# sefffal/Octofitter.jl

Hardware: AMD Instinct MI355X
Metric: epoch-likelihood evals/sec (fwd+grad), 1e4 epochs x 1e4 walkers (higher is better)
Workload: dtype f64; 1 GPU; config3: 1 planet, 10000 RA/Dec epochs x 10000 walkers in total (10000 walkers split over 1 GPUs: 10000 walkers/GPU), fwd+reverse-grad, inputs and outputs resident in HBM (PCIe-inclusive rate: value_pcie_inclusive); walkers_per_gpu=10000, walkers_total=10000, rows=10000, parallelism=walkers sharded x1, dataset replicated, no data-path collective

## Files before the change

### __graft_entry__.py

```python
from __future__ import annotations

import functools
import importlib.util
import os
import shutil
import subprocess
import sys
from pathlib import Path

ROOT = Path(__file__).resolve().parent
PKG_DIR = ROOT / "octofitter.jl_amd"
PKG_NAME = "octofitter_jl_amd"
CSRC = PKG_DIR / "csrc"
LIB = PKG_DIR / "lib" / "liboctofitter_hip.so"

HIPCC_FLAGS = [
    "--offload-arch=gfx950", "-O3", "-std=c++17", "-fPIC",
    "-ffp-contract=on",
    "-fno-gpu-rdc",
    "-mllvm", "-structurizecfg-skip-uniform-regions",
    "-Wall", "-Wno-unused-function",
]


# ... 25 lines not shown
    return all(Path(s).stat().st_mtime <= t for s in sources)


def build_hip(force=False):
    from concurrent.futures import ThreadPoolExecutor
    hipcc = shutil.which("hipcc") or "/opt/rocm/bin/hipcc"
    sources = sorted(CSRC.glob("*.hip"))
    headers = sorted(CSRC.glob("*.h")) + [ROOT / "include" / "octofitter_hip.h"]
    LIB.parent.mkdir(parents=True, exist_ok=True)
    objdir = CSRC / "build"
    objdir.mkdir(exist_ok=True)
    cflags = [f for f in HIPCC_FLAGS if f != "-shared"]

    def compile_one(src):
        obj = objdir / (src.stem + ".o")
        if not force and _newer(obj, [src] + headers):
            return obj
        subprocess.run([hipcc, *cflags, f"-I{ROOT / 'include'}", f"-I{CSRC}", "-c", "-o", str(obj), str(src)], check=True)
        return obj

    with ThreadPoolExecutor(max_workers=min(len(sources), os.cpu_count() or 1)) as ex:
        objs = list(ex.map(compile_one, sources))
    if force or not _newer(LIB, objs):
        subprocess.run([hipcc, "--offload-arch=gfx950", "-shared", "-fPIC", "-fno-gpu-rdc", "-o", str(LIB), *map(str, objs)], check=True)
    return LIB


COMPANIONS = {
    "draws": dict(header="octofitter_hip_draws.h", links_main=True, main_headers=True),
    "predict": dict(header="octofitter_hip_predict.h", links_main=True, main_headers=True),
    "pointwise": dict(header="octofitter_hip_pointwise.h", links_main=True, main_headers=True),
    "psis": dict(header="octofitter_hip_psis.h", links_main=False, main_headers=False),
}


def companion_lib(name) -> Path:
    return PKG_DIR / "lib" / f"liboctofitter_hip_{name}.so"


def build_companion(name, force=False):
    row = COMPANIONS[name]
    hipcc = shutil.which("hipcc") or "/opt/rocm/bin/hipcc"
    src_dir, shared, out = CSRC / name, CSRC / "companion", companion_lib(name)
    sources = sorted(src_dir.glob("*.hip"))
    headers = sorted(src_dir.glob("*.h")) + sorted(shared.glob("*.h")) + (sorted(CSRC.glob("*.h")) if row["main_headers"] else []) + \
        [ROOT / "include" / "octofitter_hip.h", ROOT / "include" / row["header"]]
    if row["links_main"] and not LIB.exists():
# ... 78 lines not shown
```

### octofitter.jl_amd/csrc/octo_api.hip

```cpp
#define OCTO_API_TU 1
#include "octo_host.h"
#include "octo_tile.h"

using namespace octo;

namespace octo {

std::atomic<uint64_t> g_dataset_serial{1};

int fail(octo_ctx* ctx, int code, const std::string& msg) {
    if (ctx) ctx->err = msg;
    return code;
}

int busy(octo_ctx* ctx, const char* what) {
    if (ctx->pending.active) return fail(ctx, OCTO_EINVAL, std::string(what) + ": an octo_eval_begin of this context has not been ended");
    return OCTO_OK;
}


DevConsts dev_consts(const octo_consts& c) {
    DevConsts d;
    d.k_yr = c.kepler_year_to_julian_day; d.yd = c.year2day_julian; d.au2m = c.au2m; d.sec2yr = c.sec2year_julian;
    d.mas_per_au_per_plx = c.rad2as / c.pc2au;
// ... 152 lines not shown
            t_o = std::min<int64_t>(std::max<int64_t>(t_o, 1), std::max<int64_t>(1, n / (rows_min * wpb)));
            const int64_t rows_per_task = (n + t_o - 1) / t_o;
            chunk = (rows_per_task + wpb - 1) / wpb;
        }
        const int64_t span = chunk * wpb;
        bool even = n > 1;
        {
            double smin = INFINITY, smax = 0.0;
            for (int64_t r = 1; r < n; ++r) { smin = std::min(smin, (double)ds->h_step[o][r]); smax = std::max(smax, (double)ds->h_step[o][r]); }
            even = even && std::isfinite(smax) && smin > 0.0 && smax - smin <= 1.0e-7 * smax;
        }
        for (int64_t r0 = 0; r0 < n; r0 += span) {
            Task t;
            std::memset(&t, 0, sizeof(t));
            t.obs = o; t.row0 = (int32_t)r0; t.nrows = (int32_t)std::min<int64_t>(span, n - r0); t.chunk = (int32_t)chunk;
            {
                double km = 0.0;
                for (int64_t r = r0; r < r0 + t.nrows; ++r)
                    if ((r - r0) % chunk != 0) km = std::max(km, (double)ds->h_step[o][r]);
                float f = (float)km;
                if ((double)f < km) f = std::nextafterf(f, INFINITY);
                t.key_max = std::isfinite(km) ? f : INFINITY;
                t.dm_uniform = (even && std::isfinite(km) && km > 0.0) ? f : 0.0f;
            }
            tt.h_tasks.push_back(t);
            double a = 0.0, b = 0.0;
            for (int64_t r = r0; r < r0 + t.nrows; ++r) { a += ds->h_rowconst_pre[o][r]; b += ds->h_rowconst_raw[o][r]; }
            cpre.push_back(a); craw.push_back(b);
        }
    }
    tt.n_tasks = (int)tt.h_tasks.size();
    {
        std::vector<int32_t> range(2 * std::max(ds->n_obs, 1), 0);
        std::vector<double> opre(std::max(ds->n_obs, 1), 0.0), oraw(std::max(ds->n_obs, 1), 0.0);
        int t = 0;
        for (int o = 0; o < ds->n_obs; ++o) {
            range[2 * o] = t;
            while (t < tt.n_tasks && tt.h_tasks[t].obs == o) { opre[o] += cpre[t]; oraw[o] += craw[t]; ++t; }
            range[2 * o + 1] = t;
        }
        HIPCHK(ctx, hipMalloc((void**)&tt.d_obs_range, sizeof(int32_t) * range.size()));
        HIPCHK(ctx, hipMalloc((void**)&tt.d_obs_const_pre, sizeof(double) * opre.size()));
        HIPCHK(ctx, hipMalloc((void**)&tt.d_obs_const_raw, sizeof(double) * oraw.size()));
        HIPCHK(ctx, hipMemcpy(tt.d_obs_range, range.data(), sizeof(int32_t) * range.size(), hipMemcpyHostToDevice));
        HIPCHK(ctx, hipMemcpy(tt.d_obs_const_pre, opre.data(), sizeof(double) * opre.size(), hipMemcpyHostToDevice));
        HIPCHK(ctx, hipMemcpy(tt.d_obs_const_raw, oraw.data(), sizeof(double) * oraw.size(), hipMemcpyHostToDevice));
// ... 192 lines not shown
        }
    }
    if (hipMalloc((void**)&ctx->d_counters, sizeof(int32_t) * SMALL_W) != hipSuccess ||
        hipMemset(ctx->d_counters, 0, sizeof(int32_t) * SMALL_W) != hipSuccess) {
        (void)hipFree(ctx->d_sctab); (void)hipStreamDestroy(ctx->stream); (void)hipEventDestroy(ctx->ev_order);
        delete ctx;
        return OCTO_ENOMEM;
    }
    if (hipHostMalloc((void**)&ctx->h_flags, sizeof(uint64_t) * (SMALL_W + 32), hipHostMallocMapped | hipHostMallocPortable | hipHostMallocCoherent) != hipSuccess) {
        (void)hipFree(ctx->d_counters); (void)hipFree(ctx->d_sctab); (void)hipStreamDestroy(ctx->stream); (void)hipEventDestroy(ctx->ev_order);
        delete ctx;
        return OCTO_ENOMEM;
    }
    std::memset(ctx->h_flags, 0, sizeof(uint64_t) * (SMALL_W + 32));
    if (const char* ev = std::getenv("OCTO_SMALL_W")) { ctx->small_w = std::min(std::max(std::atoi(ev), 0), SMALL_W); ctx->small_w_model = 0; }
    if (const char* ev = std::getenv("OCTO_MAPPED_W")) ctx->mapped_w = std::min(std::max(std::atoi(ev), 0), SMALL_W);
    if (const char* ev = std::getenv("OCTO_FLAG_W")) ctx->flag_w = std::min(std::max(std::atoi(ev), 0), SMALL_W);
    ctx->env_small_blocks = env_int("OCTO_SMALL_BLOCKS"); ctx->env_small_min_span = env_int("OCTO_SMALL_MIN_SPAN");
    ctx->env_stage_bytes = env_int("OCTO_STAGE_BYTES"); ctx->env_chunk = env_int("OCTO_CHUNK"); ctx->env_rounds = env_int("OCTO_ROUNDS"); ctx->env_rv_cost = env_int("OCTO_RV_COST"); ctx->env_kind_all = env_int("OCTO_KIND_ALL"); ctx->env_mainp_tpb = env_int("OCTO_MAINP_TPB");
    if (const char* ev = std::getenv("OCTO_WIDE")) ctx->env_wide = std::atoi(ev);
    if (const char* ev = std::getenv("OCTO_FIN_FUSED")) ctx->env_no_fin_fused = std::atoi(ev) ? 0 : 1;
    if (const char* ev = std::getenv("OCTO_WARM")) { ctx->env_warm = std::atoi(ev); ctx->opt_warm = ctx->env_warm ? 1 : 0; }
    if (const char* ev = std::getenv("OCTO_WARM_NEWTON")) ctx->env_warm_newton = std::atoi(ev) ? 1 : 0;
    if (const char* ev = std::getenv("OCTO_WARM_NEWTON_MID")) ctx->env_warm_newton_mid = std::atoi(ev) ? 1 : 0;
    if (const char* ev = std::getenv("OCTO_TILE_SORT")) ctx->tile_mode = std::min(std::max(std::atoi(ev), 0), 2);
    if (const char* ev = std::getenv("OCTO_TILE_MIN_W")) ctx->tile_min_w = std::max<int64_t>(std::atoll(ev), 64);
    *out = ctx;
    return OCTO_OK;
}

int32_t octo_ctx_destroy(octo_ctx* ctx) {
    if (!ctx) return OCTO_OK;
    (void)hipSetDevice(ctx->device);
    if (ctx->comm) (void)octo_comm_destroy(ctx);
    (void)hipDeviceSynchronize();
    if (ctx->stream) (void)hipStreamDestroy(ctx->stream);
    if (ctx->ev_order) (void)hipEventDestroy(ctx->ev_order);
    free_retired(ctx);
    for (auto& t : ctx->tables) free_table(t);
    for (auto& e : ctx->ev_pool) { (void)hipEventDestroy(e.first); (void)hipEventDestroy(e.second); }
    (void)hipFree(ctx->d_wc); (void)hipFree(ctx->d_valid); (void)hipFree(ctx->d_partials); (void)hipFree(ctx->d_marg); (void)hipFree(ctx->d_sctab); (void)hipFree(ctx->d_extra); (void)hipFree(ctx->d_counters);
    (void)hipHostFree(ctx->h_in); (void)hipHostFree(ctx->h_out); (void)hipHostFree(ctx->h_flags);
    (void)hipFree(ctx->d_in); (void)hipFree(ctx->d_out);
    (void)hipFree(ctx->d_perm); (void)hipHostFree(ctx->h_tile_stats);
    for (void* q : ctx->retired_host) (void)hipHostFree(q);
    if (ctx->ev_tile) (void)hipEventDestroy(ctx->ev_tile);
// ... 61 lines not shown
        case OCTO_OPT_TILE_SORT: *value_out = ctx->tile_mode; return OCTO_OK;
        case OCTO_OPT_TILE_MIN_WALKERS: *value_out = ctx->tile_min_w; return OCTO_OK;
        default: return OCTO_EINVAL;
    }
}

int32_t octo_dataset_create(octo_ctx* ctx, const octo_obs_desc* obs, int32_t n_obs,
                            const octo_planet_desc* planets, int32_t n_planets, octo_dataset** out) {
    if (!ctx || !out || n_obs < 0 || (n_obs > 0 && !obs) || !planets) return fail(ctx, OCTO_EINVAL, "octo_dataset_create: null argument");
    *out = nullptr;
    if (n_planets < 1) return fail(ctx, OCTO_EINVAL, "octo_dataset_create: a dataset needs at least one planet");
    if (n_planets > MAXP) return fail(ctx, OCTO_ENOTSUP, "octo_dataset_create: 1.." + std::to_string(MAXP) + " planets supported");
    for (int p = 0; p < n_planets; ++p)
        if (planets[p].orbit_kind != OCTO_ORBIT_VISUAL_KEP && planets[p].orbit_kind != OCTO_ORBIT_RADVEL &&
            planets[p].orbit_kind != OCTO_ORBIT_THIELE_INNES && planets[p].orbit_kind != OCTO_ORBIT_KEP)
            return fail(ctx, OCTO_EINVAL, "octo_dataset_create: unknown orbit kind");
    HIPCHK(ctx, hipSetDevice(ctx->device));
    octo_dataset* ds = new (std::nothrow) octo_dataset();
    if (!ds) return fail(ctx, OCTO_ENOMEM, "octo_dataset_create: host allocation failed");
    ds->device = ctx->device; ds->n_obs = n_obs; ds->n_planets = n_planets;
    ds->serial = g_dataset_serial.fetch_add(1);
    for (int p = 0; p < n_planets; ++p) ds->planets[p] = planets[p];
    auto bail = [&](int code, const std::string& msg) { octo_dataset_destroy(ds); return fail(ctx, code, msg); };
    ds->h_obs.resize(n_obs); ds->h_rowconst_pre.resize(n_obs); ds->h_rowconst_raw.resize(n_obs); ds->h_step.resize(n_obs);
    for (int o = 0; o < n_obs; ++o) {
        const octo_obs_desc& d = obs[o];
        if (d.kind < 0 || d.kind >= OCTO_N_KINDS) return bail(OCTO_EINVAL, "octo_dataset_create: unknown observation kind");
        if (d.n_epochs < 0 || d.n_epochs > 0x7fffffff) return bail(OCTO_EINVAL, "octo_dataset_create: bad n_epochs");
        if (d.kind == OCTO_HGCA) {
            if (d.n_epochs > 0 && (!d.epoch || !d.y1 || !d.y2)) return bail(OCTO_EINVAL, "octo_dataset_create: missing column");
            if (!d.extra || d.n_extra != OCTO_HGCA_N_EXTRA) return bail(OCTO_EINVAL, "octo_dataset_create: OCTO_HGCA needs extra[15]");
            for (int p = 0; p < n_planets; ++p)
                if (planets[p].orbit_kind != OCTO_ORBIT_RADVEL && planets[p].orbit_kind != OCTO_ORBIT_KEP && !planets[p].has_mass)
                    return bail(OCTO_EINVAL, "octo_dataset_create: OCTO_HGCA needs a mass on every Visual{KepOrbit} / ThieleInnesOrbit planet");
            for (int k = 0; k < 3; ++k)
                if (!(d.extra[5 * k + 2] > 0.0) || !(d.extra[5 * k + 3] > 0.0) || !(std::fabs(d.extra[5 * k + 4]) < 1.0))
                    return bail(OCTO_EINVAL, "octo_dataset_create: OCTO_HGCA covariance is not positive definite");
            const int64_t n = d.n_epochs;
            std::vector<double> raw((size_t)std::max<int64_t>(n, 1) * ROW_STRIDE, 0.0);
            for (int64_t r = 0; r < n; ++r) {
                const int ax = (int)d.y1[r], ms = (int)d.y2[r];
                if ((ax != OCTO_HGCA_RA && ax != OCTO_HGCA_DEC) || (ms != OCTO_HGCA_HIP && ms != OCTO_HGCA_GAIA))
                    return bail(OCTO_EINVAL, "octo_dataset_create: OCTO_HGCA rows need y1 in {RA, DEC}, y2 in {HIP, GAIA}");
                if (!std::isfinite(d.epoch[r])) return bail(OCTO_EINVAL, "octo_dataset_create: OCTO_HGCA epochs must be finite");
                raw[(size_t)r * ROW_STRIDE] = d.epoch[r]; raw[(size_t)r * ROW_STRIDE + 1] = ax; raw[(size_t)r * ROW_STRIDE + 2] = ms;
            }
            DevObs& h = ds->h_obs[o];
// ... 55 lines not shown
                if (d.cor && !(std::fabs(c) <= 1.0 - 1e-5))
                    return bail(OCTO_EINVAL, "octo_dataset_create: correlation values may not be well-specified");
                a[2] = b[2] = d.y2[r]; a[3] = s1; a[4] = s2; a[5] = c;
                const double omc = 1.0 - c * c;
                b[3] = 1.0 / (s1 * s1 * omc); b[4] = 1.0 / (s2 * s2 * omc); b[5] = -c / (s1 * s2 * omc);
                ds->h_rowconst_pre[o][r] = -LOG2PI - 0.5 * std::log(s1 * s1 * s2 * s2 * omc);
                ds->h_rowconst_raw[o][r] = -LOG2PI;
            } else {
                const double s = d.s1[r];
                a[2] = s; b[2] = 1.0 / (s * s);
                if (has_basis) {
                    if (!std::isfinite(d.extra[r])) return bail(OCTO_EINVAL, "octo_dataset_create: table " + std::to_string(o) + " row " + std::to_string(r) + ": trend basis must be finite");
                    a[3] = d.extra[r];
                }
                if (d.kind == OCTO_RV_ABS_MARG) {
                    ds->h_rowconst_pre[o][r] = -std::log(TWO_PI * s * s);
                    ds->h_rowconst_raw[o][r] = 0.0;
                } else {
                    ds->h_rowconst_pre[o][r] = -0.5 * (LOG2PI + std::log(s * s));
                    ds->h_rowconst_raw[o][r] = -0.5 * LOG2PI;
                }
            }
        }
        double dm_max = 0.0;
        std::vector<double> steps;
        steps.reserve((size_t)std::max<int64_t>(n, 1));
        for (int64_t r = 0; r < n; ++r) {
            const double dm = r > 0 ? TWO_PI * (d.epoch[r] - d.epoch[r - 1]) : 0.0;
            double key = std::fabs(dm);
            if (r > 0) { dm_max = std::max(dm_max, key); steps.push_back(key); }
            ds->h_step[o][r] = std::isfinite(key) ? key : INFINITY;
            if (r == 0 || (r % WARM_RESTART) == 0 || !std::isfinite(key)) key = INFINITY;
            raw[(size_t)r * ROW_STRIDE + 6] = pre[(size_t)r * ROW_STRIDE + 6] = dm;
            raw[(size_t)r * ROW_STRIDE + 7] = pre[(size_t)r * ROW_STRIDE + 7] = key;
        }
        DevObs& h = ds->h_obs[o];
        h.kind = d.kind; h.planet = planet_obs ? d.planet : -1; h.has_cor = d.cor ? 1 : 0; h.dm_max = ctx->env_warm ? (float)(dm_max * 1.000001) : 0.0f; h.n = n;
        for (int k = 0; k < WARM_LADDER; ++k) h.dm_ladder[k] = 0.0f;
        if (ctx->env_warm && !steps.empty()) {
            std::sort(steps.begin(), steps.end());
            static const double q[WARM_LADDER] = {0.97, 0.90, 0.75, 0.50, 0.25, 0.10, 0.03, 0.01};
            int m = 0;
            for (int k = 0; k < WARM_LADDER; ++k) {
                const size_t idx = (size_t)std::min<double>((double)steps.size() - 1.0, std::ceil(q[k] * (double)steps.size()) - 1.0 < 0.0 ? 0.0 : std::ceil(q[k] * (double)steps.size()) - 1.0);
                const double v = steps[idx];
                if (!(v > 0.0) || !std::isfinite(v)) continue;
                float f = (float)v;
                if ((double)f < v) f = std::nextafterf(f, INFINITY);
                if (m > 0 && h.dm_ladder[m - 1] == f) continue;
                h.dm_ladder[m++] = f;
            }
        }
        h.raw = h.pre = nullptr;
        if (n > 0) {
            double *dr = nullptr, *dp = nullptr;
            const size_t bytes = sizeof(double) * (size_t)n * ROW_STRIDE;
            if (hipMalloc((void**)&dr, bytes) != hipSuccess) return bail(OCTO_ENOMEM, "octo_dataset_create: hipMalloc failed");
            ds->d_bufs.push_back(dr);
// ... 37 lines not shown

static int eval_impl(octo_ctx* ctx, const octo_dataset* ds, const double* d_elems, const double* d_nuis, int64_t ld, int64_t W,
                     double* d_ll, double* d_g_elems, double* d_g_nuis, hipStream_t st, const SmallModel* sm, bool grad, bool nuis,
                     const octo_ctx::ModelTail* mt = nullptr, bool* tail_applied = nullptr) {
    ctx->mt_applied = false;
    if (tail_applied) *tail_applied = false;
    if (ctx->timing_every > 0 && ctx->ev_used >= 4096) { int rc = drain_timing(ctx); if (rc) return rc; }
    const int64_t ldw = (W + WAVE - 1) / WAVE * WAVE;
    if (ldw > ctx->cap_w) {
        int64_t need = ldw;
        if (ctx->d_wc) { ctx->retired.push_back(ctx->d_wc); ctx->d_wc = nullptr; }
        if (ctx->d_valid) { ctx->retired.push_back(ctx->d_valid); ctx->d_valid = nullptr; }
        need += need / 2;
        HIPCHK(ctx, hipMalloc((void**)&ctx->d_wc, sizeof(double) * (size_t)need * NWC * MAXP));
        HIPCHK(ctx, hipMalloc((void**)&ctx->d_valid, sizeof(int32_t) * (size_t)need * MAXP));
        ctx->cap_w = need;
    }
    EvalArgs a;
    std::memset(&a, 0, sizeof(a));
    a.obs = ds->d_obs;
    a.n_obs = ds->n_obs; a.n_planets = ds->n_planets;
    for (int p = 0; p < ds->n_planets; ++p) { a.orbit_kind[p] = ds->planets[p].orbit_kind; a.has_mass[p] = ds->planets[p].has_mass; }
    a.elems = d_elems; a.nuis = d_nuis; a.ld = ld; a.W = W;
    a.warm = (ctx->opt_warm && !ctx->opt_invariant) ? (1 | (ctx->env_warm_newton ? 2 : 0) | (ctx->env_warm_newton_mid ? 4 : 0)) : 0;
    a.ws_in = a.ws_out = 1;
    if (ctx->stage_ws_in > 0) { a.ws_in = ctx->stage_ws_in; a.ws_out = ctx->stage_ws_out; }
    a.wc = ctx->d_wc; a.valid = ctx->d_valid; a.ldw = ctx->cap_w; a.sctab = ctx->d_sctab;
    a.ll_out = d_ll; a.g_elems = d_g_elems; a.g_nuis = d_g_nuis;
    if (mt) {
        a.mt_Jc = mt->Jc; a.mt_gtp = mt->gtp; a.mt_esrc = mt->esrc; a.mt_nsrc = mt->nsrc; a.mt_glp = mt->glp; a.mt_lpp = mt->lpp; a.mt_lp = mt->lp; a.mt_grad = mt->grad;
        a.mt_ld = mt->ld; a.mt_ldo = mt->ldo; a.mt_D = mt->D; a.mt_n_nu = mt->n_nu;
    }
    a.c = dev_consts(ctx->consts);
    int rc;
    switch (ds->n_planets) {
        case 1: rc = dispatch1<1>(ctx, ds, a, grad, nuis, sm, st); break;
        case 2: rc = dispatch1<2>(ctx, ds, a, grad, nuis, sm, st); break;
        case 3: rc = dispatch1<3>(ctx, ds, a, grad, nuis, sm, st); break;
        case 4: rc = dispatch1<4>(ctx, ds, a, grad, nuis, sm, st); break;
        default: rc = dispatch_many(ctx, ds, a, grad, nuis, sm, st); break;
    }
    if (tail_applied) *tail_applied = rc == OCTO_OK && mt != nullptr && ctx->mt_applied;
    return rc;
}

int32_t octo_eval_device(octo_ctx* ctx, const octo_dataset* cds, const double* d_elems, const double* d_nuis,
                         int64_t ld, int64_t W, double* d_ll, double* d_g_elems, double* d_g_nuis, void* hip_stream) {
// ... 848 lines not shown
```

### octofitter.jl_amd/csrc/octo_device.h

```cpp
#pragma once
#include <hip/hip_runtime.h>
#include <stdint.h>

namespace octo {

constexpr int WAVE = 64;
constexpr double PI = 3.141592653589793238462643383279502884;
constexpr double TWO_PI = 6.283185307179586476925286766559005768;
constexpr double PI2 = PI * PI;
constexpr double LOG2PI = 1.8378770664093454835606594728112;
constexpr double MK_K0 = 3.0 * PI2 / (PI2 - 6.0);
constexpr double MK_K1N = 8.0 * PI / (5.0 * (PI2 - 6.0));

enum : int {
    WC_INVP = 0,
    WC_TP,
    WC_E,
    WC_BETA,
    WC_EOB,
    WC_CB, WC_CG, WC_CA, WC_CF,
    WC_K,
    WC_COSW, WC_SINW,
    WC_MU,
    WC_A,
// ... 358 lines not shown
#ifndef OCTO_WARM_NEWTON_DEPTH
#define OCTO_WARM_NEWTON_DEPTH 4
#endif
constexpr int WARM_NEWTON_DEPTH = OCTO_WARM_NEWTON_DEPTH;
static_assert(WARM_NEWTON_DEPTH == 3 || WARM_NEWTON_DEPTH == 4, "kepler_warm_newton: three or four values of history");
struct KWarmNewton {
    float c[WARM_NEWTON_DEPTH];
    float tau;
    float tau2;
    int n;
};

__device__ __forceinline__ void warm_newton_init(KWarmNewton& wn, float e, bool mid) {
    const float t = __builtin_amdgcn_sqrtf(WARM_NEWTON_TOL * __builtin_amdgcn_sqrtf(fmaf(-e, e, 1.0f)) * __builtin_amdgcn_rcpf(e));
    wn.tau = fminf(t, WARM_NEWTON_CAP);
    const float k = fmaf(0.5f * e * e, __builtin_amdgcn_rcpf(fmaf(-e, e, 1.0f)), (e * (1.0f / 6.0f)) * __builtin_amdgcn_rcpf(1.0f - e));
    const float t2 = __builtin_amdgcn_exp2f((1.0f / 3.0f) * __builtin_amdgcn_logf(WARM_NEWTON_MID_TOL * __builtin_amdgcn_rcpf(k)));
    wn.tau2 = mid ? fminf(t2, WARM_NEWTON_MID_CAP) : 0.0f;
#pragma unroll
    for (int k = 0; k < WARM_NEWTON_DEPTH; ++k) wn.c[k] = 0.0f;
    wn.n = 0;
}

template <int INV_NR, int PH = 0>
__device__ __forceinline__ KSol kepler_warm_newton(double t, const PC& pc, const SinCosTab& tab, KWarm& st, KWarmNewton& wn, double thr, double dm, const WarmPin& pin) {
    static_assert(INV_NR == 1, "kepler_warm_newton: 1/(1 − e cos E) one Newton step from the reciprocal of f1 (the adjoints' bar)");
    static_assert(PH >= 0 && PH < 4, "kepler_warm_newton: four phases");
    constexpr bool RING = WARM_NEWTON_DEPTH == 4;
    constexpr int I0 = RING ? (0 - PH) & 3 : 0, I1 = RING ? (1 - PH) & 3 : 1, I2 = RING ? (2 - PH) & 3 : 2, I3 = (3 - PH) & 3;
    KSol s;
    s.dt = t - pc.tp;
    s.E = 0.0;
    const bool apriori = __builtin_amdgcn_ballot_w64(st.invD >= thr) == 0;
    const float gate = __uint_as_float(wn.n >= WARM_NEWTON_DEPTH ? 0x3f800000u : 0u);
    float cp;
    if constexpr (WARM_NEWTON_DEPTH == 3) cp = gate * fmaf(3.0f, wn.c[0] - wn.c[1], wn.c[2]);
    else cp = gate * fmaf(4.0f, wn.c[I0] + wn.c[I2], fmaf(-6.0f, wn.c[I1], -wn.c[I3]));
    const double dM = dm * pc.invP;
    const double x = dM * st.invD;
    const double z = x * st.invD;
    const double dE = fma(-((pc.he * st.sE) * z), x, x) + (double)cp;
    const double u = dE * dE;
    const double sr = dE * fma(u, fma(u, fma(u, OCTO_KT[22], pin.k17), OCTO_KT[18]), 1.0);
    const double cm1 = u * fma(u, fma(u, fma(u, OCTO_KT[23], pin.k19), OCTO_KT[20]), -0.5);
    const double ds = fma(st.sE, cm1, st.cE * sr);
    const double s1 = st.sE + ds;
    const double c1 = fma(st.cE, cm1, fma(-st.sE, sr, st.cE));
    const double f0 = fma(-pc.e, ds, dE - dM);
    const double f1 = fma(-pc.e, c1, 1.0);
    const double r1 = rcp_nr<1>(f1);
    const double d = -f0 * r1;
    const float df = (float)d;
    s.sE = fma(c1, d, s1);
    s.cE = fma(-s1, d, c1);
    s.invD = fma(fma(-fma(-pc.e, s.cE, 1.0), r1, 1.0), r1, r1);
    float cn = cp + df;
    int n = wn.n + 1;
    const bool fast = apriori && __builtin_amdgcn_ballot_w64(fabsf(df) > wn.tau) == 0;
    if (__builtin_expect(!fast, 0)) {
        if (apriori && __builtin_amdgcn_ballot_w64(fabsf(df) > wn.tau2) == 0) {
            const double q = (pc.he * s1) * r1;
            const double dh = fma(-(q * d), d, d);
            const double w = -0.5 * dh;
            s.sE = fma(dh, fma(w, s1, c1), s1);
            s.cE = fma(dh, fma(w, c1, -s1), c1);
            const double D = fma(-pc.e, s.cE, 1.0);
            const double r2 = fma(fma(-D, r1, 1.0), r1, r1);
            s.invD = fma(fma(-D, r2, 1.0), r2, r2);
            cn = cp + (float)dh;
        } else if (apriori && __builtin_amdgcn_ballot_w64(fabsf(df) > (float)WARM_TOL) == 0) {
            double d4;
            kepler_correct<INV_NR, true>(s, pc, 0.0, s1, c1, f0, &d4);
            cn = cp + (float)d4;
        } else {
            const double uo = s.dt * pc.invP;
            const double frac = uo - rint(uo);
            const float E1f = markley_starter_f32(frac, pc);
            const double E1 = (double)E1f;
            double sc, cc;
            sincos_table(E1f, tab, sc, cc);
            kepler_correct<INV_NR>(s, pc, E1, sc, cc, fma(-pc.e, sc, fma(-frac, TWO_PI, E1)));
            cn = 0.0f;
            n = 0;
        }
    }
    if constexpr (RING) wn.c[I3] = cn;
    else {
#pragma unroll
        for (int k = WARM_NEWTON_DEPTH - 1; k > 0; --k) wn.c[k] = wn.c[k - 1];
        wn.c[0] = cn;
    }
    wn.n = n < WARM_NEWTON_DEPTH ? n : WARM_NEWTON_DEPTH;
    st.sE = s.sE; st.cE = s.cE; st.invD = s.invD;
    return s;
}

}
```

### octofitter.jl_amd/csrc/octo_host.h

```cpp
#pragma once
#include <hip/hip_runtime.h>

#include <algorithm>
#include <atomic>
#include <cmath>
#include <cstdio>
#include <cstdlib>
#include <cstring>
#include <map>
#include <mutex>
#include <new>
#include <string>
#include <vector>

#include "octo_kernels.h"
#include "octo_model.h"
#include "octo_hgca.h"
#include "octo_small.h"
#include "octofitter_hip.h"

namespace octo {

struct TaskTable {
    uint64_t ds_serial = 0;
// ... 3 lines not shown
    int n_tasks = 0;
    Task* d_tasks = nullptr;
    double* d_const_pre = nullptr;
    double* d_const_raw = nullptr;
    int32_t* d_obs_range = nullptr;
    double* d_obs_const_pre = nullptr, *d_obs_const_raw = nullptr;
    std::vector<Task> h_tasks;
};


}

using namespace octo;

struct octo_dataset {
    int device = 0;
    int n_obs = 0, n_planets = 0;
    int kind_mask = 0;
    int64_t n_rows = 0;
    int n_hgca = 0;
    std::vector<DevObs> h_obs;
    std::vector<std::vector<double>> h_rowconst_pre, h_rowconst_raw;
    std::vector<std::vector<double>> h_step;
    DevObs* d_obs = nullptr;
    std::vector<double*> d_bufs;
    octo_planet_desc planets[MAXP];
    float tile_dm_ref = 0.0f;
    int64_t tile_rows = 0;
    uint64_t serial = 0;
};

struct octo_ofti {
    int device = 0;
    int64_t n = 0;
    double* d_rows = nullptr;
    double lambda = 0, data_quad = 0, log_det_data_cov = 0, log_det_prior_inv = 0, n_log2pi = 0;
};

struct octo_ctx {
    int device = 0;
    int n_cus = 256;
    int64_t max_lds = 65536;
    hipStream_t stream = nullptr;
    hipStream_t last_stream = nullptr;
    bool has_last = false;
    hipEvent_t ev_order = nullptr;
// ... 8 lines not shown
    int64_t cap_extra = 0;
    double* d_sctab = nullptr;
    int32_t* d_counters = nullptr;
    uint64_t* h_flags = nullptr;
    uint64_t flag_seq = 0;
    bool flag_request = false, flag_armed = false;
    SmallInline inl = {};
    int64_t stage_ws_in = 0, stage_ws_out = 0;
    struct ModelTail { const double *Jc = nullptr, *gtp = nullptr, *glp = nullptr, *lpp = nullptr; const octo_source *esrc = nullptr, *nsrc = nullptr; double *lp = nullptr, *grad = nullptr; int64_t ld = 0, ldo = 0; int32_t D = 0, n_nu = 0; };
    bool mt_applied = false;
    struct Pending {
        bool active = false, staged = false, walker_major = false;
        int64_t W = 0, ld = 0, ldd = 0, ws_out = 0, o_ge = 0, o_gn = 0;
        int n_el_out = 0, n_nu_out = 0;
        double *ll = nullptr, *g_elems = nullptr, *g_nuis = nullptr;
    } pending;
    void* comm = nullptr;
    int comm_rank = 0, comm_world = 1;
    int small_w_model = 768;
    int small_w = OCTO_SMALL_BATCH_DEFAULT;
    int64_t env_small_blocks = 0, env_small_min_span = 0, env_stage_bytes = 0, env_chunk = 0, env_rounds = 0, env_rv_cost = 0, env_kind_all = 0, env_mainp_tpb = 0;
    int env_warm = 1;
    int env_warm_newton = 1;
    int env_warm_newton_mid = 1;
    int opt_warm = 1;
    int opt_invariant = 0;
    int tile_mode = 2;
    int64_t tile_min_w = 2048;
    int32_t* d_perm = nullptr; int64_t cap_perm = 0;
    float* h_tile_stats = nullptr; int64_t cap_tile_stats = 0;
    hipEvent_t ev_tile = nullptr;
    bool tile_on = false, tile_pending = false;
    int tile_pending_segs = 0;
    int64_t tile_seq = 0, tile_W = 0, tile_sorted_launches = 0, tile_probes = 0;
    uint64_t tile_ds = 0;
    double tile_last_saving_us = 0.0;
    int env_no_fin_fused = 0;
    int env_wide = 0;
    int flag_w = 128;
    int mapped_w = 128;
    double *d_in = nullptr, *d_out = nullptr;
    int64_t cap_in = 0, cap_out = 0;
    double *h_in = nullptr, *h_out = nullptr;
    int64_t cap_hin = 0, cap_hout = 0;
    std::vector<void*> retired_host;
    std::vector<void*> retired;
// ... 77 lines not shown
```

### octofitter.jl_amd/csrc/octo_kernels.h

```cpp
#pragma once
#include <type_traits>

#include "octo_device.h"
#include "octofitter_hip.h"

namespace octo {

constexpr int MAXP = OCTO_MAX_PLANETS;
constexpr int MAXP_T = OCTO_MAX_PLANETS_ALL_KINDS;
constexpr int ROW_STRIDE = 8;
constexpr int WPB = 4;
#ifndef OCTO_FIN_G
#define OCTO_FIN_G 16
#endif
#ifndef OCTO_FIN_UNROLL
#define OCTO_FIN_UNROLL 4
#endif
constexpr int FIN_G = OCTO_FIN_G;
constexpr int fin_nwr(int n_planets) { return n_planets == 2 ? 3 : (n_planets == 3 ? 2 : 1); }
#ifndef OCTO_FIN_CH
#define OCTO_FIN_CH 6
#endif
#ifndef OCTO_FIN_FAST
#define OCTO_FIN_FAST true
#endif
constexpr int FIN_CH = OCTO_FIN_CH;

constexpr int KM_RADEC = 1, KM_SEPPA = 2, KM_RVABS = 4, KM_MARG = 8, KM_RVREL = 16, KM_COR = 32, KM_ONEIL = 64;
constexpr int KM_RV = KM_RVABS | KM_MARG | KM_RVREL;
constexpr int KM_ALL = 127;
constexpr int KM_HGCA = 128;

struct DevObs {
    int32_t kind, planet, has_cor;
    float dm_max;
    int64_t n;
    const double* raw;
    const double* pre;
    float dm_ladder[WARM_LADDER];
};

struct Task {
    int32_t obs, row0, nrows, chunk;
    float key_max;
    float dm_uniform;
    int32_t pad[2];
};

struct DevConsts {
    double k_yr, yd, au2m, sec2yr, mas_per_au_per_plx , mjup2msol;
};

struct EvalArgs {
    const DevObs* obs;
    const Task* tasks;
    const double* task_const;
    const int32_t* obs_range;
    const double* obs_const;
    int32_t n_obs, n_tasks, n_planets, n_hblocks;
    int32_t warm, fin_fused;
    int32_t task0, n_rblocks;
    int32_t orbit_kind[MAXP];
    int32_t has_mass[MAXP];
    const double* elems;
    const double* nuis;
    int64_t ld, W;
    int64_t ws_in, ws_out;
    double* wc;
    int32_t* valid;
    double* partials;
// ... 302 lines not shown
        sincos_reduced(c.na, c.sn, c.cn);
        c.j2 = c.jit * c.jit;
    }
    c.seppa = (KM & KM_SEPPA) && (ob_kind == OCTO_ASTROM_SEPPA || ob_kind == OCTO_ONEIL_SEPPA);
    c.oneil = L::HAS_ONEIL && (ob_kind == OCTO_ONEIL_RADEC || ob_kind == OCTO_ONEIL_SEPPA);
    c.planet = ob_planet; c.has_cor = ob_has_cor;
    return c;
}

template <int P, bool GRAD, bool NUIS, int KM>
__device__ __forceinline__ AstromCoef<P> astrom_coef(const double* __restrict__ nuis, int64_t ld, int ob_kind, int ob_planet, int ob_has_cor,
                                                     int obs_index, const PC (&pc)[P], int64_t wl) {
    double jit = 0.0, ps = 1.0, na = 0.0;
    if constexpr (NUIS) {
        const double* nu = nuis + (int64_t)obs_index * OCTO_N_NUIS * ld + wl;
        jit = nu[OCTO_NU_JITTER * ld]; ps = nu[OCTO_NU_PLATESCALE * ld]; na = nu[OCTO_NU_NORTHANGLE * ld];
    }
    return astrom_coef_vals<P, GRAD, NUIS, KM>(jit, ps, na, ob_kind, ob_planet, ob_has_cor, pc);
}

template <int P>
struct WarmState { KWarm st[P]; double thr[P]; uint32_t key_hi; bool row_ok; WarmPin pin; };

template <int P, bool GRAD, bool NUIS, int KM, bool TAB, int WARM = 0, bool WCHECK = true, int WLAST = 0, int WPH = 0, bool WPIN = false>
__device__ __forceinline__ void astrom_row(AccArr<P, GRAD, NUIS, KM>& acc, LogProd& lp, const PC (&pc)[P],
                                           const AstromCoef<P>& co, double t, double y1, double y2, double c3, double c4, double c5,
                                           const SinCosTab& tab, WarmState<P>* ws = nullptr, double dm = 0.0, KWarmNewton* wn = nullptr) {
    using L = Layout<P, GRAD, NUIS, KM>;
    constexpr bool DEFER = TAB;
    const double (&f)[P] = co.f;
    const double jit = co.jit, j2 = co.j2, ps = co.ps, na = co.na, sn = co.sn, cn = co.cn;
    const bool seppa = co.seppa, oneil = co.oneil;
    KSol s[P];
    double rap[P], dep[P];
    double ra_m, dec_m;
#pragma unroll
    for (int p = 0; p < P; ++p) {
        if constexpr (WARM == 3) s[p] = kepler_warm_newton<1, WPH>(t, pc[p], tab, ws->st[p], *wn, ws->thr[p], dm, ws->pin);
        else if constexpr (WARM != 0) s[p] = kepler_solve_warm<1, WARM == 1, WPIN>(t, pc[p], tab, ws->st[p], ws->thr[p], dm, WCHECK ? ws->row_ok : true, &ws->pin);
        else if constexpr (WLAST != 0) { if (p == P - 1) s[p] = kepler_warm_step<1>(t, pc[p], ws->st[p], dm); else s[p] = kepler_solve<1, TAB>(t, pc[p], tab); }
        else s[p] = kepler_solve<1, TAB>(t, pc[p], tab);
        if constexpr (WLAST == 2) {
            if (p == P - 1 && __builtin_expect(!ws->row_ok, 0)) {
                s[p] = kepler_solve<1, TAB>(t, pc[p], tab);
                ws->st[p].sE = s[p].sE; ws->st[p].cE = s[p].cE; ws->st[p].invD = s[p].invD;
            }
        }
        rap[p] = fma(pc[p].cB, s[p].cE, fma(pc[p].cGb, s[p].sE, -pc[p].cBe));
        dep[p] = fma(pc[p].cA, s[p].cE, fma(pc[p].cFb, s[p].sE, -pc[p].cAe));
    }
    if constexpr (L::HAS_ONEIL) {
        if (oneil) {
            double sE = 0.0, cE = 0.0, ee = 0.0, invD = 0.0, dtp = 0.0;
#pragma unroll
            for (int p = 0; p < P; ++p) {
                const bool me = (P == 1) || (p == co.planet);
                sE = me ? s[p].sE : sE; cE = me ? s[p].cE : cE; ee = me ? pc[p].e : ee; invD = me ? s[p].invD : invD; dtp = me ? s[p].dt : dtp;
            }
            double E = 0.0;
#pragma unroll
            for (int p = 0; p < P; ++p) E = ((P == 1) || (p == co.planet)) ? s[p].E : E;
// ... 90 lines not shown
            deb = (rhob * dec_m - pab * ra_m * irho) * irho;
        } else {
            rab = -g1; deb = -g2;
        }
#pragma unroll
        for (int p = 0; p < P; ++p) {
            double* g = &acc[L::OFF_PL + p * L::PL_N];
            const double ra_f = (P == 1 || DEFER) ? rab : f[p] * rab, de_f = (P == 1 || DEFER) ? deb : f[p] * deb;
            g[L::U1] = fma(s[p].cE, ra_f, g[L::U1]);
            g[L::U2] = fma(s[p].sE, ra_f, g[L::U2]);
            g[L::U3] = fma(s[p].cE, de_f, g[L::U3]);
            g[L::U4] = fma(s[p].sE, de_f, g[L::U4]);
            g[L::U5] += ra_f;
            g[L::U6] += de_f;
            if constexpr (P > 1) {
                if constexpr (DEFER) g[L::GC] += fma(rab, rap[p], deb * dep[p]);
                else g[L::GC] += (p == co.planet) ? 0.0 : ((f[p] != 0.0) ? fma(rab, rap[p], deb * dep[p]) : 0.0);
            }
            const double dra = fma(pc[p].cGb, s[p].cE, -(pc[p].cB * s[p].sE));
            const double dde = fma(pc[p].cFb, s[p].cE, -(pc[p].cA * s[p].sE));
            const double Mb = fma(ra_f, dra, de_f * dde) * s[p].invD;
            g[L::GE] = fma(Mb, s[p].sE, g[L::GE]);
            g[L::GM] += Mb;
            g[L::GT] = fma(Mb, s[p].dt, g[L::GT]);
        }
    }
}

template <int P>
struct RvCoef {
    double gc[P];
    double gK[P];
    double ib2[P];
    double off, jit, j2, mu_hat, iA;
    double trend;
    bool rel, marg;
    int planet;
};

template <int P, bool GRAD, bool NUIS, int KM>
__device__ __forceinline__ RvCoef<P> rv_coef_vals(double off, double jit, double trend, const double* __restrict__ margp, int64_t ldw,
                                                  int ob_kind, int ob_planet, int obs_index, const PC (&pc)[P], int64_t wl) {
    RvCoef<P> c;
    c.rel = (KM & KM_RVREL) && ob_kind == OCTO_RV_REL;
    {
        double a_this = 0.0;
#pragma unroll
        for (int p = 0; p < P; ++p) a_this = (p == ob_planet) ? pc[p].a : a_this;
// ... 217 lines not shown
}

#ifndef OCTO_WARM
#define OCTO_WARM 1
#endif
#ifndef OCTO_WARM_PLAIN
#define OCTO_WARM_PLAIN 0
#endif
template <int P, bool GRAD, bool NUIS, int KM, bool FUSED>
constexpr bool main_warm_plain() {
    return OCTO_WARM && FUSED && P == 1 && !(KM & KM_ONEIL) && NUIS && ((KM & KM_SEPPA) || ((KM & KM_RV) && OCTO_WARM_PLAIN));
}
template <int P, bool GRAD, bool NUIS, int KM, bool FUSED>
constexpr bool main_warm() {
    return OCTO_WARM && FUSED && P == 1 && !(KM & KM_ONEIL);
}
#ifndef OCTO_WARM_NEWTON
#define OCTO_WARM_NEWTON 1
#endif
template <int P, bool GRAD, bool NUIS, int KM, bool FUSED, int NWV, bool FINF>
constexpr bool main_warm_newton() {
    return OCTO_WARM_NEWTON && main_warm<P, GRAD, NUIS, KM, FUSED>() && !main_warm_plain<P, GRAD, NUIS, KM, FUSED>() && !NUIS && NWV == WPB && !FINF &&
           (KM == KM_RADEC || KM == (KM_RADEC | KM_COR));
}

#ifndef OCTO_WARM_PIN
#define OCTO_WARM_PIN 1
#endif
template <int P, bool GRAD, bool NUIS, int KM, bool FUSED, int NWV, bool FINF>
constexpr bool main_warm_pin() {
    return main_warm_newton<P, GRAD, NUIS, KM, FUSED, NWV, FINF>() ||
           (OCTO_WARM_PIN && main_warm<P, GRAD, NUIS, KM, FUSED>() && !main_warm_plain<P, GRAD, NUIS, KM, FUSED>() && !NUIS && NWV == WPB && !FINF);
}

#ifndef OCTO_WARM_LAST3
#define OCTO_WARM_LAST3 1
#endif
template <int P, bool GRAD, bool NUIS, int KM, bool FUSED>
constexpr bool main_warm_last() {
    return OCTO_WARM && FUSED && (P == 2 || (P == 3 && OCTO_WARM_LAST3 && !(KM & KM_SEPPA))) && !(KM & (KM_ONEIL | KM_MARG));
}

template <int P>
__device__ __forceinline__ float warm_last_init(WarmState<P>& ws, const PC& pc, const DevObs& ob, bool enabled) {
    float bound = 0.0f;
#pragma unroll
// ... 195 lines not shown
                constexpr bool WPIN = main_warm_pin<P, GRAD, NUIS, KM, FUSED, NWV, FINF>();
                if constexpr (WPIN) ws.pin = warm_pin();
                auto wbody_t = [&](const RowRegs8& r, auto checked) {
                    if constexpr (decltype(checked)::value) ws.row_ok = warm_row_ok<P>(ws, r);
                    astrom_row<P, GRAD, NUIS, KM, true, WMODE, decltype(checked)::value, 0, 0, WPIN>(acc, lp, pc, co, row_get(r, 0), row_get(r, 1), row_get(r, 2),
                                                                                                     row_get(r, 3), row_get(r, 4), row_get(r, 5), tab, &ws, row_get(r, 6));
                };
                auto wloop = [&](auto checked) {
                    RowRegs8 A = row_issue8(rows);
                    for (int j = 0; j < n_rows; j += 2) {
                        RowRegs8 B = row_wait_issue(A, rows + (int64_t)(j + 1 < n_rows ? j + 1 : j) * ROW_STRIDE);
                        wbody_t(A, checked);
                        if (__builtin_expect(j + 1 >= n_rows, 0)) { row_drain(B); break; }
                        A = row_wait_issue(B, rows + (int64_t)(j + 2 < n_rows ? j + 2 : j + 1) * ROW_STRIDE);
                        wbody_t(B, checked);
                    }
                    row_drain(A);
                };
                if constexpr (main_warm_newton<P, GRAD, NUIS, KM, FUSED, NWV, FINF>()) {
                    if (n_rows > 0) {
                        if (warm_unchecked && (a.warm & 2) != 0 && tk.dm_uniform > 0.0f) {
                            KWarmNewton wn;
                            warm_newton_init(wn, pc[0].ef, (a.warm & 4) != 0);
                            auto nbody = [&](const RowRegs8& r, auto ph) {
                                astrom_row<P, GRAD, NUIS, KM, true, 3, false, 0, decltype(ph)::value>(acc, lp, pc, co, row_get(r, 0), row_get(r, 1), row_get(r, 2),
                                                                                                      row_get(r, 3), row_get(r, 4), row_get(r, 5), tab, &ws, row_get(r, 6), &wn);
                            };
                            const int skip = (4 - (n_rows & 3)) & 3;
                            auto row_at = [&](int k) { k -= skip; return rows + (int64_t)(k < 0 ? 0 : (k < n_rows ? k : n_rows - 1)) * ROW_STRIDE; };
                            RowRegs8 A = row_issue8(rows);
                            for (int j = 0;; j += 4) {
                                RowRegs8 B = row_wait_issue(A, row_at(j + 1));
                                if (__builtin_expect(j >= skip, 1)) nbody(A, std::integral_constant<int, 0>{});
                                A = row_wait_issue(B, row_at(j + 2));
                                if (__builtin_expect(j + 1 >= skip, 1)) nbody(B, std::integral_constant<int, 1>{});
                                B = row_wait_issue(A, row_at(j + 3));
                                if (__builtin_expect(j + 2 >= skip, 1)) nbody(A, std::integral_constant<int, 2>{});
                                A = row_wait_issue(B, row_at(j + 4));
                                nbody(B, std::integral_constant<int, 3>{});
                                if (j + 4 >= n_rows + skip) break;
                            }
                            row_drain(A);
                        } else wloop(std::true_type{});
                    }
                } else if (n_rows > 0) {
                    if (warm_unchecked) wloop(std::false_type{});
                    else wloop(std::true_type{});
                }
            }
        } else if (n_rows > 0) {
            RowRegs A = row_issue(rows);
            for (int j = 0; j < n_rows; j += 2) {
                RowRegs B = row_wait_issue(A, rows + (int64_t)(j + 1 < n_rows ? j + 1 : j) * ROW_STRIDE);
                body(A);
                if (__builtin_expect(j + 1 >= n_rows, 0)) { row_drain(B); break; }
                A = row_wait_issue(B, rows + (int64_t)(j + 2 < n_rows ? j + 2 : j + 1) * ROW_STRIDE);
                body(B);
            }
            row_drain(A);
        }
        astrom_finish_sums<P, GRAD, NUIS, KM>(acc, co);
    }
    if (L::HAS_RV && !is_astrom) {
        const RvCoef<P> co = rv_coef<P, GRAD, NUIS, KM>(a.nuis, a.ld, a.marg, a.ldw, ob.kind, ob.planet, tk.obs, pc, wsrc);
        const crow_t rows = constant_rows((NUIS ? ob.raw : ob.pre) + (int64_t)row_first * ROW_STRIDE);
// ... 871 lines not shown
```

Baseline: 403.6 billion evals/s.

## Specialize warm Newton loop for exactly evenly spaced epochs

On the host, each observation is checked for exactly uniform epoch spacing, and the exact mean-anomaly step is stored in the task. When it is present, the warm-Newton loop uses a hoisted constant dM instead of a per-row load and multiply, and it issues 7-wide rather than 8-wide row loads. In mode 2 it also drops the per-row dt computation and the time-of-periastron gradient FMA, keeping a running sum and applying a closed-form correction at the end. This lowers per-row ALU work and register pressure, at the cost of a different floating-point summation order for the tp gradient and an extra exactness check when the dataset is built.

```diff
diff --git a/__graft_entry__.py b/__graft_entry__.py
--- a/__graft_entry__.py
+++ b/__graft_entry__.py
@@ -71,7 +71,7 @@
     with ThreadPoolExecutor(max_workers=min(len(sources), os.cpu_count() or 1)) as ex:
         objs = list(ex.map(compile_one, sources))
     if force or not _newer(LIB, objs):
-        subprocess.run([hipcc, "--offload-arch=gfx950", "-shared", "-fPIC", "-fno-gpu-rdc", "-o", str(LIB), *map(str, objs)], check=True)
+        subprocess.run([hipcc, "--offload-arch=gfx950", "-shared", "-fPIC", "-fno-gpu-rdc", "-s", "-o", str(LIB), *map(str, objs)], check=True)
     return LIB
 
 
diff --git a/octofitter.jl_amd/csrc/octo_api.hip b/octofitter.jl_amd/csrc/octo_api.hip
--- a/octofitter.jl_amd/csrc/octo_api.hip
+++ b/octofitter.jl_amd/csrc/octo_api.hip
@@ -198,6 +198,7 @@
                 if ((double)f < km) f = std::nextafterf(f, INFINITY);
                 t.key_max = std::isfinite(km) ? f : INFINITY;
                 t.dm_uniform = (even && std::isfinite(km) && km > 0.0) ? f : 0.0f;
+                t.dm_exact = t.dm_uniform > 0.0f ? ds->h_dm_exact[o] : 0.0;
             }
             tt.h_tasks.push_back(t);
             double a = 0.0, b = 0.0;
@@ -436,6 +437,7 @@
     if (const char* ev = std::getenv("OCTO_FIN_FUSED")) ctx->env_no_fin_fused = std::atoi(ev) ? 0 : 1;
     if (const char* ev = std::getenv("OCTO_WARM")) { ctx->env_warm = std::atoi(ev); ctx->opt_warm = ctx->env_warm ? 1 : 0; }
     if (const char* ev = std::getenv("OCTO_WARM_NEWTON")) ctx->env_warm_newton = std::atoi(ev) ? 1 : 0;
+    if (const char* ev = std::getenv("OCTO_WARM_EVEN")) ctx->env_warm_even = std::atoi(ev) <= 0 ? 0 : (std::atoi(ev) == 1 ? 1 : 2);
     if (const char* ev = std::getenv("OCTO_WARM_NEWTON_MID")) ctx->env_warm_newton_mid = std::atoi(ev) ? 1 : 0;
     if (const char* ev = std::getenv("OCTO_TILE_SORT")) ctx->tile_mode = std::min(std::max(std::atoi(ev), 0), 2);
     if (const char* ev = std::getenv("OCTO_TILE_MIN_W")) ctx->tile_min_w = std::max<int64_t>(std::atoll(ev), 64);
@@ -543,7 +545,7 @@
     ds->serial = g_dataset_serial.fetch_add(1);
     for (int p = 0; p < n_planets; ++p) ds->planets[p] = planets[p];
     auto bail = [&](int code, const std::string& msg) { octo_dataset_destroy(ds); return fail(ctx, code, msg); };
-    ds->h_obs.resize(n_obs); ds->h_rowconst_pre.resize(n_obs); ds->h_rowconst_raw.resize(n_obs); ds->h_step.resize(n_obs);
+    ds->h_obs.resize(n_obs); ds->h_rowconst_pre.resize(n_obs); ds->h_rowconst_raw.resize(n_obs); ds->h_step.resize(n_obs); ds->h_dm_exact.assign(n_obs, 0.0);
     for (int o = 0; o < n_obs; ++o) {
         const octo_obs_desc& d = obs[o];
         if (d.kind < 0 || d.kind >= OCTO_N_KINDS) return bail(OCTO_EINVAL, "octo_dataset_create: unknown observation kind");
@@ -645,11 +647,18 @@
                 }
             }
         }
-        double dm_max = 0.0;
+        double dm_max = 0.0, dm_exact = 0.0;
+        bool exact = n > 1;
         std::vector<double> steps;
         steps.reserve((size_t)std::max<int64_t>(n, 1));
         for (int64_t r = 0; r < n; ++r) {
             const double dm = r > 0 ? TWO_PI * (d.epoch[r] - d.epoch[r - 1]) : 0.0;
+            if (r > 0) {
+                const double ta = d.epoch[r], tb = d.epoch[r - 1], h = ta - tb, h1 = d.epoch[1] - d.epoch[0];
+                const double bb = h - ta, err = (ta - (h - bb)) + (-tb - bb);
+                if (r == 1) dm_exact = dm;
+                exact = exact && std::isfinite(dm) && h > 0.0 && err == 0.0 && std::memcmp(&h, &h1, sizeof(double)) == 0 && std::memcmp(&dm, &dm_exact, sizeof(double)) == 0;
+            }
             double key = std::fabs(dm);
             if (r > 0) { dm_max = std::max(dm_max, key); steps.push_back(key); }
             ds->h_step[o][r] = std::isfinite(key) ? key : INFINITY;
@@ -657,6 +666,7 @@
             raw[(size_t)r * ROW_STRIDE + 6] = pre[(size_t)r * ROW_STRIDE + 6] = dm;
             raw[(size_t)r * ROW_STRIDE + 7] = pre[(size_t)r * ROW_STRIDE + 7] = key;
         }
+        ds->h_dm_exact[o] = exact ? dm_exact : 0.0;
         DevObs& h = ds->h_obs[o];
         h.kind = d.kind; h.planet = planet_obs ? d.planet : -1; h.has_cor = d.cor ? 1 : 0; h.dm_max = ctx->env_warm ? (float)(dm_max * 1.000001) : 0.0f; h.n = n;
         for (int k = 0; k < WARM_LADDER; ++k) h.dm_ladder[k] = 0.0f;
@@ -740,7 +750,7 @@
     a.n_obs = ds->n_obs; a.n_planets = ds->n_planets;
     for (int p = 0; p < ds->n_planets; ++p) { a.orbit_kind[p] = ds->planets[p].orbit_kind; a.has_mass[p] = ds->planets[p].has_mass; }
     a.elems = d_elems; a.nuis = d_nuis; a.ld = ld; a.W = W;
-    a.warm = (ctx->opt_warm && !ctx->opt_invariant) ? (1 | (ctx->env_warm_newton ? 2 : 0) | (ctx->env_warm_newton_mid ? 4 : 0)) : 0;
+    a.warm = (ctx->opt_warm && !ctx->opt_invariant) ? (1 | (ctx->env_warm_newton ? 2 : 0) | (ctx->env_warm_newton_mid ? 4 : 0) | (ctx->env_warm_even >= 1 ? 8 : 0) | (ctx->env_warm_even >= 2 ? 16 : 0)) : 0;
     a.ws_in = a.ws_out = 1;
     if (ctx->stage_ws_in > 0) { a.ws_in = ctx->stage_ws_in; a.ws_out = ctx->stage_ws_out; }
     a.wc = ctx->d_wc; a.valid = ctx->d_valid; a.ldw = ctx->cap_w; a.sctab = ctx->d_sctab;
diff --git a/octofitter.jl_amd/csrc/octo_device.h b/octofitter.jl_amd/csrc/octo_device.h
--- a/octofitter.jl_amd/csrc/octo_device.h
+++ b/octofitter.jl_amd/csrc/octo_device.h
@@ -404,21 +404,24 @@
     wn.n = 0;
 }
 
-template <int INV_NR, int PH = 0>
+template <int INV_NR, int PH = 0, bool HOIST = false, bool NODT = false>
 __device__ __forceinline__ KSol kepler_warm_newton(double t, const PC& pc, const SinCosTab& tab, KWarm& st, KWarmNewton& wn, double thr, double dm, const WarmPin& pin) {
     static_assert(INV_NR == 1, "kepler_warm_newton: 1/(1 − e cos E) one Newton step from the reciprocal of f1 (the adjoints' bar)");
     static_assert(PH >= 0 && PH < 4, "kepler_warm_newton: four phases");
     constexpr bool RING = WARM_NEWTON_DEPTH == 4;
     constexpr int I0 = RING ? (0 - PH) & 3 : 0, I1 = RING ? (1 - PH) & 3 : 1, I2 = RING ? (2 - PH) & 3 : 2, I3 = (3 - PH) & 3;
     KSol s;
-    s.dt = t - pc.tp;
+    if constexpr (NODT) s.dt = 0.0;
+    else s.dt = t - pc.tp;
     s.E = 0.0;
     const bool apriori = __builtin_amdgcn_ballot_w64(st.invD >= thr) == 0;
     const float gate = __uint_as_float(wn.n >= WARM_NEWTON_DEPTH ? 0x3f800000u : 0u);
     float cp;
     if constexpr (WARM_NEWTON_DEPTH == 3) cp = gate * fmaf(3.0f, wn.c[0] - wn.c[1], wn.c[2]);
     else cp = gate * fmaf(4.0f, wn.c[I0] + wn.c[I2], fmaf(-6.0f, wn.c[I1], -wn.c[I3]));
-    const double dM = dm * pc.invP;
+    double dM;
+    if constexpr (HOIST) dM = dm;
+    else dM = dm * pc.invP;
     const double x = dM * st.invD;
     const double z = x * st.invD;
     const double dE = fma(-((pc.he * st.sE) * z), x, x) + (double)cp;
@@ -455,7 +458,10 @@
             kepler_correct<INV_NR, true>(s, pc, 0.0, s1, c1, f0, &d4);
             cn = cp + (float)d4;
         } else {
-            const double uo = s.dt * pc.invP;
+            double dtc;
+            if constexpr (NODT) dtc = t - pc.tp;
+            else dtc = s.dt;
+            const double uo = dtc * pc.invP;
             const double frac = uo - rint(uo);
             const float E1f = markley_starter_f32(frac, pc);
             const double E1 = (double)E1f;
diff --git a/octofitter.jl_amd/csrc/octo_host.h b/octofitter.jl_amd/csrc/octo_host.h
--- a/octofitter.jl_amd/csrc/octo_host.h
+++ b/octofitter.jl_amd/csrc/octo_host.h
@@ -49,6 +49,7 @@
     std::vector<DevObs> h_obs;
     std::vector<std::vector<double>> h_rowconst_pre, h_rowconst_raw;
     std::vector<std::vector<double>> h_step;
+    std::vector<double> h_dm_exact;
     DevObs* d_obs = nullptr;
     std::vector<double*> d_bufs;
     octo_planet_desc planets[MAXP];
@@ -103,6 +104,7 @@
     int64_t env_small_blocks = 0, env_small_min_span = 0, env_stage_bytes = 0, env_chunk = 0, env_rounds = 0, env_rv_cost = 0, env_kind_all = 0, env_mainp_tpb = 0;
     int env_warm = 1;
     int env_warm_newton = 1;
+    int env_warm_even = 2;
     int env_warm_newton_mid = 1;
     int opt_warm = 1;
     int opt_invariant = 0;
diff --git a/octofitter.jl_amd/csrc/octo_kernels.h b/octofitter.jl_amd/csrc/octo_kernels.h
--- a/octofitter.jl_amd/csrc/octo_kernels.h
+++ b/octofitter.jl_amd/csrc/octo_kernels.h
@@ -44,8 +44,9 @@
     int32_t obs, row0, nrows, chunk;
     float key_max;
     float dm_uniform;
-    int32_t pad[2];
+    double dm_exact;
 };
+static_assert(sizeof(Task) == 32, "Task: eight dwords, two scalar loads");
 
 struct DevConsts {
     double k_yr, yd, au2m, sec2yr, mas_per_au_per_plx , mjup2msol;
@@ -394,7 +395,7 @@
 template <int P>
 struct WarmState { KWarm st[P]; double thr[P]; uint32_t key_hi; bool row_ok; WarmPin pin; };
 
-template <int P, bool GRAD, bool NUIS, int KM, bool TAB, int WARM = 0, bool WCHECK = true, int WLAST = 0, int WPH = 0, bool WPIN = false>
+template <int P, bool GRAD, bool NUIS, int KM, bool TAB, int WARM = 0, bool WCHECK = true, int WLAST = 0, int WPH = 0, bool WPIN = false, int WEVEN = 0>
 __device__ __forceinline__ void astrom_row(AccArr<P, GRAD, NUIS, KM>& acc, LogProd& lp, const PC (&pc)[P],
                                            const AstromCoef<P>& co, double t, double y1, double y2, double c3, double c4, double c5,
                                            const SinCosTab& tab, WarmState<P>* ws = nullptr, double dm = 0.0, KWarmNewton* wn = nullptr) {
@@ -408,7 +409,7 @@
     double ra_m, dec_m;
 #pragma unroll
     for (int p = 0; p < P; ++p) {
-        if constexpr (WARM == 3) s[p] = kepler_warm_newton<1, WPH>(t, pc[p], tab, ws->st[p], *wn, ws->thr[p], dm, ws->pin);
+        if constexpr (WARM == 3) s[p] = kepler_warm_newton<1, WPH, (WEVEN >= 1), (WEVEN >= 2)>(t, pc[p], tab, ws->st[p], *wn, ws->thr[p], dm, ws->pin);
         else if constexpr (WARM != 0) s[p] = kepler_solve_warm<1, WARM == 1, WPIN>(t, pc[p], tab, ws->st[p], ws->thr[p], dm, WCHECK ? ws->row_ok : true, &ws->pin);
         else if constexpr (WLAST != 0) { if (p == P - 1) s[p] = kepler_warm_step<1>(t, pc[p], ws->st[p], dm); else s[p] = kepler_solve<1, TAB>(t, pc[p], tab); }
         else s[p] = kepler_solve<1, TAB>(t, pc[p], tab);
@@ -545,8 +546,19 @@
             const double Mb = fma(ra_f, dra, de_f * dde) * s[p].invD;
             g[L::GE] = fma(Mb, s[p].sE, g[L::GE]);
             g[L::GM] += Mb;
-            g[L::GT] = fma(Mb, s[p].dt, g[L::GT]);
-        }
+            if constexpr (WEVEN >= 2) g[L::GT] += g[L::GM];
+            else g[L::GT] = fma(Mb, s[p].dt, g[L::GT]);
+        }
+    }
+}
+
+template <int P, bool GRAD, bool NUIS, int KM>
+__device__ __forceinline__ void even_gt_finish(AccArr<P, GRAD, NUIS, KM>& acc, const PC (&pc)[P], double t_last, double h) {
+    using L = Layout<P, GRAD, NUIS, KM>;
+    static_assert(P == 1, "even_gt_finish: the single-planet Newton-only loop");
+    if constexpr (GRAD) {
+        double* g = &acc[L::OFF_PL];
+        g[L::GT] = fma(-h, g[L::GT], ((t_last - pc[0].tp) + h) * g[L::GM]);
     }
 }
 
@@ -810,6 +822,14 @@
 constexpr bool main_warm_newton() {
     return OCTO_WARM_NEWTON && main_warm<P, GRAD, NUIS, KM, FUSED>() && !main_warm_plain<P, GRAD, NUIS, KM, FUSED>() && !NUIS && NWV == WPB && !FINF &&
            (KM == KM_RADEC || KM == (KM_RADEC | KM_COR));
+}
+
+#ifndef OCTO_WARM_EVEN
+#define OCTO_WARM_EVEN 2
+#endif
+template <int P, bool GRAD, bool NUIS, int KM, bool FUSED, int NWV, bool FINF>
+constexpr int main_warm_even() {
+    return main_warm_newton<P, GRAD, NUIS, KM, FUSED, NWV, FINF>() ? OCTO_WARM_EVEN : 0;
 }
 
 #ifndef OCTO_WARM_PIN
@@ -1051,25 +1071,45 @@
                         if (warm_unchecked && (a.warm & 2) != 0 && tk.dm_uniform > 0.0f) {
                             KWarmNewton wn;
                             warm_newton_init(wn, pc[0].ef, (a.warm & 4) != 0);
-                            auto nbody = [&](const RowRegs8& r, auto ph) {
-                                astrom_row<P, GRAD, NUIS, KM, true, 3, false, 0, decltype(ph)::value>(acc, lp, pc, co, row_get(r, 0), row_get(r, 1), row_get(r, 2),
-                                                                                                      row_get(r, 3), row_get(r, 4), row_get(r, 5), tab, &ws, row_get(r, 6), &wn);
-                            };
                             const int skip = (4 - (n_rows & 3)) & 3;
                             auto row_at = [&](int k) { k -= skip; return rows + (int64_t)(k < 0 ? 0 : (k < n_rows ? k : n_rows - 1)) * ROW_STRIDE; };
-                            RowRegs8 A = row_issue8(rows);
-                            for (int j = 0;; j += 4) {
-                                RowRegs8 B = row_wait_issue(A, row_at(j + 1));
-                                if (__builtin_expect(j >= skip, 1)) nbody(A, std::integral_constant<int, 0>{});
-                                A = row_wait_issue(B, row_at(j + 2));
-                                if (__builtin_expect(j + 1 >= skip, 1)) nbody(B, std::integral_constant<int, 1>{});
-                                B = row_wait_issue(A, row_at(j + 3));
-                                if (__builtin_expect(j + 2 >= skip, 1)) nbody(A, std::integral_constant<int, 2>{});
-                                A = row_wait_issue(B, row_at(j + 4));
-                                nbody(B, std::integral_constant<int, 3>{});
-                                if (j + 4 >= n_rows + skip) break;
-                            }
-                            row_drain(A);
+                            auto nloop = [&](auto even, auto issue) {
+                                constexpr int EV = decltype(even)::value;
+                                double dmh = 0.0;
+                                if constexpr (EV >= 1) dmh = tk.dm_exact * pc[0].invP;
+                                auto nbody = [&](const auto& r, auto ph) {
+                                    double dm;
+                                    if constexpr (EV >= 1) dm = dmh;
+                                    else dm = row_get(r, 6);
+                                    astrom_row<P, GRAD, NUIS, KM, true, 3, false, 0, decltype(ph)::value, false, EV>(acc, lp, pc, co, row_get(r, 0), row_get(r, 1), row_get(r, 2),
+                                                                                                                     row_get(r, 3), row_get(r, 4), row_get(r, 5), tab, &ws, dm, &wn);
+                                };
+                                auto A = issue(rows);
+                                for (int j = 0;; j += 4) {
+                                    auto B = row_wait_issue(A, row_at(j + 1));
+                                    if (__builtin_expect(j >= skip, 1)) nbody(A, std::integral_constant<int, 0>{});
+                                    A = row_wait_issue(B, row_at(j + 2));
+                                    if (__builtin_expect(j + 1 >= skip, 1)) nbody(B, std::integral_constant<int, 1>{});
+                                    B = row_wait_issue(A, row_at(j + 3));
+                                    if (__builtin_expect(j + 2 >= skip, 1)) nbody(A, std::integral_constant<int, 2>{});
+                                    A = row_wait_issue(B, row_at(j + 4));
+                                    nbody(B, std::integral_constant<int, 3>{});
+                                    if (j + 4 >= n_rows + skip) break;
+                                }
+                                row_drain(A);
+                                if constexpr (EV >= 2 && GRAD) {
+                                    const double t_last = rows[(int64_t)(n_rows - 1) * ROW_STRIDE];
+                                    const double h = n_rows > 1 ? t_last - rows[(int64_t)(n_rows - 2) * ROW_STRIDE] : 0.0;
+                                    even_gt_finish<P, GRAD, NUIS, KM>(acc, pc, t_last, h);
+                                }
+                            };
+                            constexpr int WEV = main_warm_even<P, GRAD, NUIS, KM, FUSED, NWV, FINF>();
+                            if (WEV != 0 && (a.warm & 8) != 0 && tk.dm_exact != 0.0 && n_rows > WARM_NEWTON_DEPTH) {
+                                if constexpr (WEV >= 2 && GRAD) {
+                                    if ((a.warm & 16) != 0) nloop(std::integral_constant<int, 2>{}, [](crow_t q) { return row_issue(q); });
+                                    else nloop(std::integral_constant<int, 1>{}, [](crow_t q) { return row_issue(q); });
+                                } else if constexpr (WEV != 0) nloop(std::integral_constant<int, WEV>{}, [](crow_t q) { return row_issue(q); });
+                            } else nloop(std::integral_constant<int, 0>{}, [](crow_t q) { return row_issue8(q); });
                         } else wloop(std::true_type{});
                     }
                 } else if (n_rows > 0) {
```

Result: faster. 412.5 billion evals/s (median of 6 runs) (+2.2%).
